# wuliwei9278/primalCR

Measured on AMD Instinct MI355X. Metric: pairwise-comparisons/sec, higher is better.
Workload: dtype f32; 1 GPU; ml1m-shaped PrimalCR++ -k 100 -l 5000 (configs[1]); 6040 users x 3952 items, 939809 ratings, 131347247 ordered pairs; 1 step = 1 outer iteration (V step + U step); solver=PrimalCR++, rank=100, parallelism=user-sharded x1, accumulation=f64, storage=f32

## Files before the change

### primalcr_amd/csrc/pcr_host.cpp

```cpp
#include "pcr_host.h"

#include <algorithm>
#include <atomic>
#include <cerrno>
#include <climits>
#include <cstdint>
#include <cmath>
#include <cstdio>
#include <cstdlib>
#include <cstring>
#include <exception>
#include <functional>
#include <limits>
#include <memory>
#include <mutex>
#include <numeric>
#include <random>
#include <thread>
#include <fcntl.h>
#include <sys/mman.h>
#include <sys/stat.h>
#include <unistd.h>

static thread_local std::string g_err;
// ... 213 lines not shown
}

static int check_test_ids(int64_t d2, int64_t tnnz, const int32_t* tuser, const int32_t* titem, int threads) {
    const int T = pieces_for(tnnz, threads);
    std::vector<int64_t> bad((size_t)T, -1);
    run_pieces(tnnz, T, [&](int t, int64_t lo, int64_t hi) {
        for (int64_t z = lo; z < hi; ++z)
            if (titem[z] < 0 || titem[z] >= d2 || tuser[z] < 0) { bad[(size_t)t] = z; return; }
    });
    for (int64_t b : bad)
        if (b >= 0) {
            pcr_set_error("test rating " + std::to_string(b) + " has user/item id outside the meta dimensions");
            return PCR_ERR_ARG;
        }
    return PCR_OK;
}

extern "C" int pcr_dataset_from_triplets(int64_t d1, int64_t d2, int64_t nnz, const int32_t* user,
                                         const int32_t* item, const double* val, int64_t tnnz,
                                         const int32_t* tuser, const int32_t* titem, const double* tval,
                                         pcr_dataset** out) {
    if (!out || d1 < 0 || d2 < 0 || nnz < 0 || tnnz < 0 || (nnz > 0 && (!user || !item || !val)) ||
        (tnnz > 0 && (!tuser || !titem || !tval))) {
        pcr_set_error("pcr_dataset_from_triplets: bad argument");
        return PCR_ERR_ARG;
    }
    if (d1 > kMaxDim || d2 > kMaxDim) { pcr_set_error("pcr_dataset_from_triplets: more than 2^31 - 2 users or items"); return PCR_ERR_UNSUPPORTED; }
    return guarded("pcr_dataset_from_triplets", [&]() -> int {
        std::unique_ptr<pcr_dataset> ds(new pcr_dataset());
        const int threads = pcr_host_threads();
        int rc = build_train_csr(d1, d2, nnz, user, item, val, ds->train, threads, false);
        if (rc != PCR_OK) return rc;
        rc = check_test_ids(d2, tnnz, tuser, titem, threads);
        if (rc != PCR_OK) return rc;
        keep_raw_test(*ds, d1, tnnz, tuser, titem, tval);
        build_test_csr(d1, d2, tnnz, tuser, titem, tval, ds->test, threads, false);
        ds->tnnz_file = tnnz;
        *out = ds.release();
        return PCR_OK;
    });
}

extern "C" int pcr_dataset_from_csr(int64_t d1, int64_t d2, const int64_t* index, const int32_t* item, const double* val,
                                    const int64_t* tindex, const int32_t* titem, const double* tval, pcr_dataset** out) {
    if (!out || d1 < 0 || d2 < 0 || !index || index[0] != 0 || (tindex && tindex[0] != 0)) {
        pcr_set_error("pcr_dataset_from_csr: bad argument");
        return PCR_ERR_ARG;
    }
    const int64_t nnz = index[d1], tnnz = tindex ? tindex[d1] : 0;
    if (nnz < 0 || tnnz < 0 || (nnz > 0 && (!item || !val)) || (tnnz > 0 && (!titem || !tval))) {
        pcr_set_error("pcr_dataset_from_csr: bad argument");
        return PCR_ERR_ARG;
    }
    for (int64_t u = 0; u < d1; ++u) {
        if (index[u + 1] < index[u] || (tindex && tindex[u + 1] < tindex[u])) { pcr_set_error("pcr_dataset_from_csr: index not monotone"); return PCR_ERR_ARG; }
        for (int64_t z = index[u]; z < index[u + 1]; ++z)
            if (item[z] < 0 || item[z] >= d2 || (z > index[u] && item[z] <= item[z - 1])) {
                pcr_set_error("pcr_dataset_from_csr: user " + std::to_string(u) + ": item ids must be ascending and inside [0, d2)");
                return PCR_ERR_ARG;
            }
    }
    for (int64_t z = 0; z < tnnz; ++z)
        if (titem[z] < 0 || titem[z] >= d2) { pcr_set_error("pcr_dataset_from_csr: test item id outside [0, d2)"); return PCR_ERR_ARG; }
    if (d1 > kMaxDim || d2 > kMaxDim) { pcr_set_error("pcr_dataset_from_csr: more than 2^31 - 2 users or items"); return PCR_ERR_UNSUPPORTED; }
    return guarded("pcr_dataset_from_csr", [&]() -> int {
        std::unique_ptr<pcr_dataset> ds(new pcr_dataset());
        ds->train.d1 = ds->test.d1 = d1; ds->train.d2 = ds->test.d2 = d2;
        ds->train.index.assign(index, index + d1 + 1);
        ds->train.item.assign(item, item + nnz);
        ds->train.val.assign(val, val + nnz);
        if (tindex) ds->test.index.assign(tindex, tindex + d1 + 1); else ds->test.index.assign(d1 + 1, 0);
        ds->test.item.assign(titem, titem + tnnz);
        ds->test.val.assign(tval, tval + tnnz);
        ds->tnnz_file = tnnz;
        *out = ds.release();
        return PCR_OK;
    });
}

#include <map>
static std::map<std::string, std::string>& tune_table() { static thread_local std::map<std::string, std::string> t; return t; }
static const char* const TUNE_KEYS[] = {"ustep_mode", "cluster_k", "cluster_users", "ubins", "ustep_gram", "spmm_tiles", "spmm_chunk", "sddmm_csc",
                                        "lanes", "pipeline", "window_cache", "prepare_merged", "resort_window", "allreduce_chunks", "p2p_ll",
                                        "p2p_timeout_ms", "p2p_queue_budget", "count_rows", "debug", "win16", "ustep_win_lds", "plan_key64", "ustep_newton", "vblock_users", "recommend_select", "ranks_batch_users", "sample_threads", "rerank_lds", "ridge_form", "nnls_form", "itemfold_table_bytes", "fault_cluster_member", "fault_p2p_skip", "fault_p2p_coarse", nullptr};
extern "C" int pcr_tune(const char* key, const char* value) {
    if (!key) { pcr_set_error("pcr_tune: null key"); return PCR_ERR_ARG; }
    bool known = false;
    for (const char* const* k = TUNE_KEYS; *k; ++k) known = known || !strcmp(*k, key);
    if (!known) { pcr_set_error(std::string("pcr_tune: unknown key '") + key + "'"); return PCR_ERR_ARG; }
    if (value) tune_table()[key] = value; else tune_table().erase(key);
    return PCR_OK;
}
bool pcr_tune_get(const char* key, std::string* out) {
    auto it = tune_table().find(key);
    if (it == tune_table().end()) return false;
    if (out) *out = it->second;
    return true;
}
int pcr_tune_int(const char* key, int dflt) {
    std::string v;
    return pcr_tune_get(key, &v) ? atoi(v.c_str()) : dflt;
}


struct TextFile {
    const char* p = nullptr;
    size_t len = 0;
    void* map = nullptr;
    size_t map_len = 0;
    pcr_vec<char> heap;
    ~TextFile() { if (map) munmap(map, map_len); }
    int open(const std::string& path) {
        const int fd = ::open(path.c_str(), O_RDONLY | O_CLOEXEC);
        if (fd < 0) { pcr_set_error("can't open " + path + ": " + strerror(errno)); return PCR_ERR_IO; }
        struct stat sb;
        if (fstat(fd, &sb) == 0 && S_ISREG(sb.st_mode) && sb.st_size > 0) {
            void* m = mmap(nullptr, (size_t)sb.st_size, PROT_READ, MAP_PRIVATE, fd, 0);
            if (m != MAP_FAILED) {
                (void)madvise(m, (size_t)sb.st_size, MADV_WILLNEED);
                map = m; map_len = (size_t)sb.st_size; p = static_cast<const char*>(m); len = map_len;
                ::close(fd);
                return PCR_OK;
            }
        }
        size_t cap = (size_t)1 << 20, got = 0;
        heap.resize(cap);
        for (;;) {
            const ssize_t n = ::read(fd, heap.data() + got, cap - got);
            if (n < 0) { if (errno == EINTR) continue; ::close(fd); pcr_set_error("can't read " + path + ": " + strerror(errno)); return PCR_ERR_IO; }
            if (n == 0) break;
            got += (size_t)n;
            if (got == cap) { cap *= 2; heap.resize(cap); }
        }
        ::close(fd);
        p = heap.data(); len = got;
        return PCR_OK;
    }
};

struct SlowCopy {
    char buf[512];
    size_t n;
    SlowCopy(const char* p, const char* end) { n = std::min<size_t>(sizeof(buf) - 1, (size_t)(end - p)); memcpy(buf, p, n); buf[n] = 0; }
};

static inline bool parse_one(const char*& p, const char* end, int32_t& u, int32_t& it, double& v) {
    auto skip_ws = [&]() { while (p < end && (*p == ' ' || *p == '\t' || *p == '\n' || *p == '\r')) ++p; };
    auto parse_uint = [&](long& out) -> bool {
        skip_ws();
        const char* s = p;
        long x = 0;
        while (p < end && *p >= '0' && *p <= '9') { if (x < ((long)1 << 40)) x = x * 10 + (*p - '0'); ++p; }
        if (p == s || (p < end && (*p == '.' || *p == '-' || *p == '+' || *p == 'e' || *p == 'E'))) { p = s; return false; }
        out = x;
        return true;
    };
    const char* save = p;
    long a, b;
    if (parse_uint(a) && parse_uint(b)) {
        skip_ws();
        const char* s = p;
        bool neg = false;
        if (p < end && (*p == '-' || *p == '+')) { neg = *p == '-'; ++p; }
        long ip = 0; int nd = 0;
        while (p < end && *p >= '0' && *p <= '9' && nd < 15) { ip = ip * 10 + (*p - '0'); ++p; ++nd; }
        bool simple = nd > 0 || (p < end && *p == '.');
        double val = (double)ip;
// ... 1714 lines not shown
```

### primalcr_amd/csrc/pcr_solver.hip

```cpp
#include <hip/hip_runtime.h>
#include <rccl/rccl.h>

#include <algorithm>
#include <chrono>
#include <cmath>
#include <cstdio>
#include <cstring>
#include <limits>
#include <memory>
#include <string>
#include <vector>

#include "pcr_host.h"
#include "pcr_dev.h"
#include "pcr_kernels.h"
#include "pcr_gram.h"
#include "pcr_newton.h"
#include "pcr_vblock.h"
#include "pcr_p2p.h"

#define NCCLCHK(expr)                                                                          \
    do {                                                                                       \
        ncclResult_t e_ = (expr);                                                              \
        if (e_ != ncclSuccess) {                                                               \
            pcr_set_error(std::string(#expr) + ": " + ncclGetErrorString(e_));                 \
            return PCR_ERR_COMM;                                                               \
        }                                                                                      \
    } while (0)
#include "pcr_plan.h"
#include "pcr_plan_dev.h"

#include "pcr_classes.h"

struct Tune {
    int lanes = 0, spmm_chunk = 0, spmm_tiles = 0, sddmm_csc = -1, ustep_mode = 0, cluster_k = 4, cluster_users = 0, window_cache = 1,
        prepare_merged = -1, pipeline = 1, debug = 0, fault_cluster_member = 0, ustep_gram = -1, count_rows = 0, allreduce_chunks = 0,
        resort_window = 8, p2p_ll = 16, p2p_timeout_ms = 20000, p2p_queue_budget = 0, fault_p2p_skip = 0, fault_p2p_coarse = 0, win16 = 1, ustep_win_lds = 1, plan_key64 = 0, ustep_newton = 0, vblock_users = 0, recommend_select = 1;
    std::string ubins;
    void read() {
        lanes = pcr_tune_int("lanes", 0); spmm_chunk = pcr_tune_int("spmm_chunk", 0); spmm_tiles = pcr_tune_int("spmm_tiles", 0);
        sddmm_csc = pcr_tune_int("sddmm_csc", -1); ustep_mode = pcr_tune_int("ustep_mode", 0); cluster_k = pcr_tune_int("cluster_k", 4);
        cluster_users = pcr_tune_int("cluster_users", 0); window_cache = pcr_tune_int("window_cache", 1);
        prepare_merged = pcr_tune_int("prepare_merged", -1);
        pipeline = pcr_tune_int("pipeline", 1); debug = pcr_tune_int("debug", 0); fault_cluster_member = pcr_tune_int("fault_cluster_member", 0);
        ustep_gram = pcr_tune_int("ustep_gram", -1); count_rows = pcr_tune_int("count_rows", 0);
        allreduce_chunks = pcr_tune_int("allreduce_chunks", 0);
        resort_window = pcr_tune_int("resort_window", 8); p2p_ll = pcr_tune_int("p2p_ll", 16);
        p2p_timeout_ms = pcr_tune_int("p2p_timeout_ms", 20000); fault_p2p_skip = pcr_tune_int("fault_p2p_skip", 0);
        fault_p2p_coarse = pcr_tune_int("fault_p2p_coarse", 0); p2p_queue_budget = pcr_tune_int("p2p_queue_budget", 0);
        win16 = pcr_tune_int("win16", 1); ustep_win_lds = pcr_tune_int("ustep_win_lds", 1); plan_key64 = pcr_tune_int("plan_key64", 0); ustep_newton = pcr_tune_int("ustep_newton", 0); vblock_users = pcr_tune_int("vblock_users", 0);
        recommend_select = pcr_tune_int("recommend_select", 1);
        ubins.clear(); pcr_tune_get("ubins", &ubins);
    }
};

template <typename T>
struct Solver final : pcr_solver {
    pcr_params prm;
    Tune tune;
    int rank = 0, nranks = 1;
    int64_t d1 = 0, d2 = 0, tnnz_file = 0;
    Geo geo;
    hipStream_t st = nullptr;
    static constexpr int NSIDE = 12;
    hipStream_t side[NSIDE] = {};
    hipEvent_t ev_fork = nullptr;
    hipStream_t hi = nullptr;
    hipEvent_t ev_hi = nullptr;
    static constexpr int MAXLANE = 8;
    hipStream_t lane[MAXLANE] = {};
    hipEvent_t ev_lane[MAXLANE] = {};
    int nlane = 1;
    int pipe_lanes = 0;
    bool hi_on_solver_pipe = false;
    std::vector<hipStream_t> hi_spare;
    ncclComm_t comm = nullptr;
    std::unique_ptr<P2PComm> p2p;
    bool single() const { return (nranks == 1 && !comm && !p2p) || local_only; }
    int ncu = 256;

    Shard<T> sh;
    DBuf<int64_t> d_uptr, d_runofs;
    DBuf<int32_t> d_sidx;
    DBuf<double> d_objr;
    DBuf<int32_t> d_item, d_c2r, d_runstart, d_sitem, d_cuser, d_crow, d_ruser, d_slot_base, d_item_slot, d_chunk_ptr, d_slot_id;
    DBuf<int2> d_blk_chunks;
    DBuf<int32_t> d_blk_user, d_cpos_dense;
    DBuf<unsigned char> d_excl;
    int vblock_nbp = 0;
    DBuf<int32_t> d_newton_users;
    DBuf<double> d_dir;
    DBuf<char> d_newton_scratch;
    int newton_n = 0, newton_cap = 0, newton_rs = 0, newton_grid = 0;
    size_t newton_stride = 0;
    DBuf<int32_t> d_cuf;
    int spmm_blocks = 0, spmm_tiles = 1;
    int n_rng = 1;
    std::vector<int64_t> rng_item;
    std::vector<int> rng_blk;
    hipStream_t ar_st = nullptr;
    std::vector<hipEvent_t> ev_rng;
    hipEvent_t ev_ar = nullptr;
    bool sddmm_csc = false;
    DBuf<T> d_slab;
    bool sweep_pf4 = false;
    int spmm_chunk = 128;
    int sddmm_tile = 0;
    DBuf<uint16_t> d_lvl, d_slvl;
    DBuf<unsigned char> d_rhint;
    DBuf<uint16_t> d_win;
    DBuf<T> d_ms, d_c, d_mcsr, d_b;
    DBuf<double> d_objp;
    std::vector<Bin> bins;
    std::vector<Bin> sbins;
    std::vector<Bin> pbins;
    std::vector<Bin> ubins;
    unsigned* bar_p = nullptr;
    size_t bar_n = 0;
    DBuf<char> d_xch;
    DBuf<unsigned long long> d_rowcnt;
    size_t xch_stride = 0;
    int max_clusters = 1;
    struct EvalSet {
        int64_t nnz = 0;
        DBuf<int64_t> uptr;
        DBuf<int32_t> item;
        DBuf<double> val, gain, idcg, disc;
        DBuf<uint16_t> elvl;
        DBuf<int64_t> erunofs;
        DBuf<int32_t> erunstart;
        int max_raw_levels = 0;
        std::vector<Bin> bins;
        std::vector<int64_t> h_uptr;
        std::vector<double> h_val;
// ... 702 lines not shown
        for (int l = 1; l < nlane; ++l)
            if (used[l]) { HIPCHK(hipEventRecord(ev_lane[l], lane[l])); RC(join(ev_lane[l])); }
        HIPCHK(hipGetLastError());
        return PCR_OK;
    }
    int join(hipEvent_t ev) {
        if (!device_join) HIPCHK(hipEventSynchronize(ev)); else HIPCHK(hipStreamWaitEvent(st, ev, 0));
        return PCR_OK;
    }
    template <class F>
    int for_ubins(F launch) {
        std::vector<Bin*> order;
        for (auto& b : ubins) if (!b.users.empty() && b.K > 1) order.push_back(&b);
        const size_t nhead = order.size();
        for (auto& b : ubins) if (!b.users.empty() && b.K <= 1) order.push_back(&b);
        if (order.empty()) return PCR_OK;
        std::stable_sort(order.begin() + nhead, order.end(), [](const Bin* a, const Bin* b) { return a->cap > b->cap; });
        std::vector<std::pair<int, int>> plan;
        {
            for (size_t i = 0; i < nhead; ++i) plan.push_back({(int)i, MAXLANE});
            std::vector<int> ring;
            for (int l = 0; l < nlane; ++l) ring.push_back(nlane >= 2 && l < 2 ? l ^ 1 : l);
            std::vector<int> tail_ring;
            for (int l : ring) if (l != 0) { tail_ring.push_back(l); if (tail_ring.size() == 1 && nhead) tail_ring.push_back(MAXLANE); }
            tail_ring.push_back(0);
            for (size_t i = nhead; i < order.size(); ++i) {
                const size_t j = i - nhead;
                plan.push_back({(int)i, j < ring.size() ? ring[j] : tail_ring[(j - ring.size()) % tail_ring.size()]});
            }
        }
        if (tune.debug && !plan_announced && (plan_announced = true))
            for (auto& pr : plan) fprintf(stderr, "[pcr] U step: %s on stream %d\n", pname("ustep", *order[pr.first]).c_str(), pr.second);
        const bool idle = hipStreamQuery(st) == hipSuccess;
        ProfScope wall(&prof, "wall:ustep", st);
        bool used[MAXLANE + 1] = {};
        if (!idle) HIPCHK(hipEventRecord(ev_fork, st));
        for (auto& pr : plan) {
            Bin& b = *order[pr.first];
            hipStream_t q = pr.second == MAXLANE ? hi : lane[pr.second];
            if (!idle && q != st && !used[pr.second]) HIPCHK(hipStreamWaitEvent(q, ev_fork, 0));
            used[pr.second] = true;
            ProfScope ps(&prof, pname("ustep", b), q, b.nnz, (int64_t)b.users.size());
            launch(b, q);
        }
        for (int l = 1; l < nlane; ++l)
            if (used[l]) { HIPCHK(hipEventRecord(ev_lane[l], lane[l])); RC(join(ev_lane[l])); }
        if (used[MAXLANE]) { HIPCHK(hipEventRecord(ev_hi, hi)); RC(join(ev_hi)); }
        HIPCHK(hipGetLastError());
        return PCR_OK;
    }
    bool plan_announced = false;
    template <class F>
    int for_bins_seq(std::vector<Bin>& bs, const char* cls, F launch) {
        for (auto& b : bs) {
            if (b.users.empty()) continue;
            ProfScope ps(&prof, pname(cls, b), st, b.nnz, (int64_t)b.users.size());
            launch(b, st);
        }
        HIPCHK(hipGetLastError());
        return PCR_OK;
    }
    std::string ustep_classes() override {
        std::string all;
        for (auto& b : ubins) if (!b.users.empty()) { if (!all.empty()) all += ","; all += pname("ustep", b); }
        return all;
    }
    int class_rows(const std::string& slot, double* v) override {
        for (size_t bi = 0; bi < ubins.size(); ++bi) {
            if (ubins[bi].users.empty() || pname("ustep", ubins[bi]) != slot) continue;
            unsigned long long x = 0;
            HIPCHK(hipStreamSynchronize(st));
            HIPCHK(hipMemcpy(&x, d_rowcnt.p + bi, sizeof x, hipMemcpyDeviceToHost));
            *v = (double)x;
            return PCR_OK;
        }
        pcr_set_error("pcr_solver_counter: no U-step class '" + slot + "'");
        return PCR_ERR_ARG;
    }
    size_t small_common(int block) const { return carve_bytes(geo.ld, sizeof(T)) + carve_bytes(block / PCR_WAVE + 1, 8); }
    int strict() const { return prm.solver_type == PCR_SOLVER_PCR ? 1 : 0; }
    int foldin_params(pcr_params* p) override { *p = prm; return PCR_OK; }
    double ridge_lambda() override { return prm.lambda; }

    int launch_sddmm(const T* M, const int32_t* rows, T* out, const int* skip = nullptr) {
        if (nnz_local == 0) return PCR_OK;
        ProfScope ps(&prof, "sddmm", st);
        const T* Umat = d_U.p;
        if (sddmm_tile == 0) {
            sddmm_tile = 64;
            int per_cu = 0;
            const int ngrp0 = 256 / geo.G;
            if (hipOccupancyMaxActiveBlocksPerMultiprocessor(&per_cu, k_sddmm<T, 256>, 256, (size_t)ngrp0 * 128 * 8) == hipSuccess && per_cu > 0) {
                const int64_t fit = cdiv(nnz_local, (int64_t)ncu * per_cu * ngrp0);
                if (fit > 64 && fit <= 128) sddmm_tile = (int)((fit + 7) / 8 * 8);
            }
        }
        const int tile = sddmm_tile;
        const int ngrp = 256 / geo.G, span = ngrp * tile;
        const int grid = cdiv(nnz_local, span);
        hipLaunchKernelGGL((k_sddmm<T, 256>), dim3(grid), dim3(256), (size_t)span * 8, st, Umat, M, d_ruser.p, rows, nnz_local, out, geo, tile, skip,
                           (const int32_t*)nullptr, (const int2*)nullptr, (const int32_t*)nullptr);
        HIPCHK(hipGetLastError());
        return PCR_OK;
    }
    bool sddmm_by_tiles() const { return sddmm_csc; }
    int launch_sddmm_csc(const T* A, T* out, const int* skip) {
        if (nnz_local == 0) return PCR_OK;
        ProfScope ps(&prof, "sddmm", st);
        const int span = (256 / geo.G) * spmm_chunk;
        hipLaunchKernelGGL((k_sddmm<T, 256>), dim3(spmm_blocks), dim3(256), (size_t)span * 8, st, A, d_U.p, d_crow.p, d_cuser.p, nnz_local, out, geo,
                           spmm_chunk, skip, d_c2r.p, d_blk_chunks.p, d_chunk_ptr.p);
        HIPCHK(hipGetLastError());
        return PCR_OK;
    }

    bool prepare_is_single_launch() const {
        const bool merged = tune.prepare_merged >= 0 ? tune.prepare_merged != 0 : nnz_local < (int64_t)4000000;
        return merged && !pbins[0].users.empty() && !pbins[1].users.empty();
    }
    int launch_prepare(const T* Vm) {
        RC(launch_sddmm(Vm, d_item.p, d_mcsr.p));
        const Shard<T>& shp = sh;
        auto fn = [&](Bin& b, hipStream_t q) {
            const int nus = (int)b.users.size();
            const int cap_pad = b.big ? host_pow2(b.cap) : b.cap, rsc = b.max_lev + 2;
            const size_t bigb = prepare_bytes<T>(b.cap, cap_pad, rsc, b.big ? 8 : 4);
            const size_t lds = small_common(b.block) + (b.big ? 0 : bigb);
            const int grid = b.big ? std::min(nus, scratch_blocks) : nus;
#define LP(BL, BG) hipLaunchKernelGGL((k_prepare<T, BL, BG>), dim3(grid), dim3(BL), lds, q, shp, geo, b.d_users.p, nus, d_mcsr.p, b.cap, cap_pad, rsc, d_scratch.p, scratch_stride, strict())
            if (b.big) LP(512, true);
            else if (b.block == 64) LP(64, false);
            else if (b.block == 256) LP(256, false);
            else LP(512, false);
#undef LP
        };
        Bin &ba = pbins[0], &bb = pbins[1];
        if (prepare_is_single_launch()) {
            const int na = (int)ba.users.size(), nb = (int)bb.users.size();
            const int cpa = ba.cap, cpb = bb.cap, rsa = ba.max_lev + 2, rsb = bb.max_lev + 2;
            const size_t wb = (small_common(64) + prepare_bytes<T>(ba.cap, cpa, rsa, 4) + 15) & ~(size_t)15;
            const int wbs = 512, wpb = wbs / 64;
            const size_t lds = std::max(wb * wpb, small_common(wbs) + prepare_bytes<T>(bb.cap, cpb, rsb, 4));
            {
                ProfScope ps(&prof, "prepare/all", st, ba.nnz + bb.nnz, (int64_t)(na + nb));
                hipLaunchKernelGGL((k_prepare_all<T, 512>), dim3(nb + cdiv(na, wpb)), dim3(512), lds, st, shp, ba.d_users.p, na, ba.cap, cpa, rsa, wb,
                                   bb.d_users.p, nb, bb.cap, cpb, rsb, nb, d_mcsr.p, strict());
            }
            if (!pbins[2].users.empty()) { ProfScope ps(&prof, pname("prepare", pbins[2]), st, pbins[2].nnz, (int64_t)pbins[2].users.size()); fn(pbins[2], st); }
            HIPCHK(hipGetLastError());
            have_sorted = true;
            sh.prev_valid = 1;
            return PCR_OK;
        }
        RC(for_bins(bins, "prepare", fn));
        have_sorted = true;
        sh.prev_valid = 1;
        return PCR_OK;
    }

    int launch_vsweep(bool hv, const T* A, const int* skip = nullptr) {
        if (hv) { if (sddmm_by_tiles()) RC(launch_sddmm_csc(A, d_b.p, skip)); else RC(launch_sddmm(A, d_sitem.p, d_b.p, skip)); }
        if (hv && vblock_nbp) {
            ProfScope ps(&prof, "vblock_b", st);
            const int64_t tiles = (int64_t)(vblock_nbp / GramMfma<T>::TS) * cdiv(d2, GramMfma<T>::TS);
#ifndef PCR_NO_OPTIONAL_KERNELS
            hipLaunchKernelGGL((k_vblock_b<T>), dim3((unsigned)cdiv(tiles, 4)), dim3(256), 0, st, d_U.p, A, d_blk_user.p, vblock_nbp, d_cpos_dense.p, d2, geo, d_b.p, skip);
#endif
            HIPCHK(hipGetLastError());
        }
        return launch_sweeps(hv, skip, hv && sddmm_by_tiles());
    }
    int launch_sweeps(bool hv, const int* skip, bool b_csr = false) {
        const int bc = (b_csr ? 1 : 0) | (sweep_pf4 ? 2 : 0);
        const bool two = hv && !sh.ws;
        const bool wt = sh.uw != nullptr;
        auto fn = [&](Bin& b, hipStream_t q) {
            const int nus = (int)b.users.size();
            const int rsc = b.max_lev + 2;
            if (b.block == 64) {
                const size_t wb = (vsweep_wave_bytes<T>(b.cap, rsc, two) + 15) & ~(size_t)15;
#define LW(HV, WT) hipLaunchKernelGGL((k_vsweep_wave<T, HV, WT>), dim3(cdiv(nus, 4)), dim3(256), wb * 4, q, sh, b.d_users.p, nus, d_b.p, d_c.p, b.cap, rsc, wb, strict(), skip, bc)
                if (hv) { if (wt) LW(true, true); else LW(true, false); } else { if (wt) LW(false, true); else LW(false, false); }
#undef LW
                return;
            }
            const size_t bigb = vsweep_bytes<T>(b.cap, rsc, two);
            const size_t lds = small_common(b.block) + (b.big ? 0 : bigb);
            const int grid = b.big ? std::min(nus, scratch_blocks) : nus;
#define LV(BL, BG, HV) do { if (wt) LVW(BL, BG, HV, true); else LVW(BL, BG, HV, false); } while (0)
#define LVW(BL, BG, HV, WT) hipLaunchKernelGGL((k_vsweep<T, BL, BG, HV, WT>), dim3(grid), dim3(BL), lds, q, sh, geo, b.d_users.p, nus, d_b.p, d_c.p, b.cap, rsc, d_scratch.p, scratch_stride, strict(), skip, bc)
            if (hv) { if (b.big) LV(512, true, true); else LV(512, false, true); }
            else { if (b.big) LV(512, true, false); else LV(512, false, false); }
#undef LVW
#undef LV
        };
        Bin &ba = sbins[0], &bb = sbins[1];
        if (!ba.users.empty() && !bb.users.empty()) {
            const int na = (int)ba.users.size(), nb = (int)bb.users.size();
            const int rsa = ba.max_lev + 2, rsb = bb.max_lev + 2;
            const size_t wb = (vsweep_wave_bytes<T>(ba.cap, rsa, two) + 15) & ~(size_t)15;
            const int wbs = 512, wpb = wbs / 64;
            const size_t lds = std::max(wb * wpb, small_common(wbs) + vsweep_bytes<T>(bb.cap, rsb, two));
            const int grid = nb + cdiv(na, wpb);
            {
                ProfScope ps(&prof, std::string(hv ? "vhv" : "vgrad") + "/all", st, ba.nnz + bb.nnz, (int64_t)(na + nb));
#define LVA(HV, WBS, MW) do { if (wt) LVAW(HV, WBS, MW, true); else LVAW(HV, WBS, MW, false); } while (0)
#define LVAW(HV, WBS, MW, WT) hipLaunchKernelGGL((k_vsweep_all<T, HV, WBS, MW, WT>), dim3(grid), dim3(WBS), lds, st, sh, ba.d_users.p, na, ba.cap, rsa, wb, \
                                        bb.d_users.p, nb, bb.cap, rsb, nb, d_b.p, d_c.p, strict(), skip, bc)
                const bool dense = lds <= (size_t)40 * 1024;
                if (hv) { if (dense) { LVA(true, 512, 8); } else { LVA(true, 512, 1); } } else { if (dense) { LVA(false, 512, 8); } else { LVA(false, 512, 1); } }
#undef LVAW
#undef LVA
            }
            if (!sbins[2].users.empty()) { ProfScope ps(&prof, pname(hv ? "vhv" : "vgrad", sbins[2]), st, sbins[2].nnz, (int64_t)sbins[2].users.size()); fn(sbins[2], st); }
            HIPCHK(hipGetLastError());
            return PCR_OK;
        }
        RC(for_bins_seq(sbins, hv ? "vhv" : "vgrad", fn));
        return PCR_OK;
    }

    int fin_blocks() const { return (int)std::min<int64_t>(1024, cdiv(d2, 256 / geo.G)); }
    int launch_spmm_range(int r, T* out, const T* base, double beta, const int* skip, const T* dots_rr) {
        if (nnz_local > 0 && rng_blk[r + 1] > rng_blk[r]) {
            ProfScope ps(&prof, "spmm", st);
            hipLaunchKernelGGL((k_spmm<T, 256>), dim3(rng_blk[r + 1] - rng_blk[r]), dim3(256), 0, st, d_c.p, d_c2r.p, d_cuf.p,
                               d_chunk_ptr.p, d_slot_base.p, d_slot_id.p, d_blk_chunks.p + rng_blk[r], d_U.p, d_slab.p, geo, skip);
        }
        const int j0 = (int)rng_item[r], j1 = (int)rng_item[r + 1];
        if (j1 <= j0) return PCR_OK;
        const int grid = n_rng == 1 ? fin_blocks() : (int)std::min<int64_t>(1024, cdiv(j1 - j0, 256 / geo.G));
        ProfScope ps2(&prof, "spmm_fin", st);
        if (dots_rr) hipLaunchKernelGGL((k_spmm_fin<T, 256, true>), dim3(grid), dim3(256), 0, st, d_slab.p, d_item_slot.p, base, beta, j1, out, geo, skip, dots_rr, d_partA.p, j0);
        else hipLaunchKernelGGL((k_spmm_fin<T, 256, false>), dim3(grid), dim3(256), 0, st, d_slab.p, d_item_slot.p, base, beta, j1, out, geo, skip, (const T*)nullptr, (double*)nullptr, j0);
        return PCR_OK;
    }
    int launch_spmm(T* out, const T* base, double beta, const int* skip = nullptr, const T* dots_rr = nullptr) {
        const size_t n = (size_t)d2 * geo.ld;
        if (n_rng == 1) {
            RC(launch_spmm_range(0, out, base, beta, skip, dots_rr));
            if (vblock_nbp) {
                ProfScope ps(&prof, "vblock_hp", st);
                const int64_t tiles = (int64_t)cdiv(d2, GramMfma<T>::TS) * cdiv(geo.ld, GramMfma<T>::TS);
#ifndef PCR_NO_OPTIONAL_KERNELS
                hipLaunchKernelGGL((k_vblock_hp<T>), dim3((unsigned)cdiv(tiles, 4)), dim3(256), 0, st, d_U.p, d_c.p, d_blk_user.p, vblock_nbp, d_cpos_dense.p, d2, geo, out, skip);
#endif
            }
            HIPCHK(hipGetLastError());
            return allreduce_T(out, n);
        }
        const bool exch = !single();
        auto queue = [&](int r) -> int {
            RC(launch_spmm_range(r, out, base, beta, skip, nullptr));
            if (exch) HIPCHK(hipEventRecord(ev_rng[r], st));
            return PCR_OK;
        };
        RC(queue(0));
        for (int r = 0; r < n_rng; ++r) {
            if (r + 1 < n_rng) RC(queue(r + 1));
            if (!exch) continue;
            HIPCHK(hipStreamWaitEvent(ar_st, ev_rng[r], 0));
            const size_t lo = (size_t)rng_item[r] * geo.ld, hi = (size_t)rng_item[r + 1] * geo.ld;
            if (hi > lo) RC(allreduce_T(out + lo, hi - lo, ar_st));
        }
        if (exch) { HIPCHK(hipEventRecord(ev_ar, ar_st)); HIPCHK(hipStreamWaitEvent(st, ev_ar, 0)); }
        HIPCHK(hipGetLastError());
        return PCR_OK;
    }

    int allreduce_T(T* buf, size_t count, hipStream_t q = nullptr) {
        if (single()) return PCR_OK;
        if (!comm && !p2p) { pcr_set_error("nranks > 1 but neither pcr_solver_comm_init nor pcr_solver_comm_init_p2p was called"); return PCR_ERR_STATE; }
        if (!q) q = st;
        ProfScope ps(&prof, "allreduce", q);
        if (p2p) {
            if (!p2p->allreduce<T>(buf, count, q)) { pcr_set_error("p2p all-reduce: " + p2p->err); return PCR_ERR_COMM; }
            return PCR_OK;
        }
        NCCLCHK(ncclAllReduce(buf, buf, count, sizeof(T) == 4 ? ncclFloat : ncclDouble, ncclSum, comm, q));
        return PCR_OK;
    }
    int allreduce_f64(double* buf, size_t count) override {
        if (single()) return PCR_OK;
        if (!comm && !p2p) { pcr_set_error("nranks > 1 but neither pcr_solver_comm_init nor pcr_solver_comm_init_p2p was called"); return PCR_ERR_STATE; }
        ProfScope ps(&prof, "allreduce", st);
        if (p2p) {
            if (!p2p->allreduce<double>(buf, count, st, true)) { pcr_set_error("p2p all-reduce: " + p2p->err); return PCR_ERR_COMM; }
            return PCR_OK;
        }
        NCCLCHK(ncclAllReduce(buf, buf, count, ncclDouble, ncclSum, comm, st));
        return PCR_OK;
    }

    int reduce_sum(const double* in, int64_t n, int slot) {
        const int nb = (int)std::min<int64_t>(512, std::max<int64_t>(1, cdiv(n, 2048)));
        const int per = cdiv(std::max<int64_t>(n, 1), nb);
        hipLaunchKernelGGL(k_sum_stage1, dim3(nb), dim3(PCR_EW_BLOCK), 0, st, in, n, per, d_partA.p);
        hipLaunchKernelGGL(k_fin2, dim3(1), dim3(PCR_EW_BLOCK), 0, st, d_partA.p, nb, d_scal.p + slot);
        HIPCHK(hipGetLastError());
        return PCR_OK;
    }
    int norm2(const T* a, int64_t n, int slot) {
        const int nb = (int)std::min<int64_t>(512, std::max<int64_t>(1, cdiv(n, 4096)));
        const int per = cdiv(std::max<int64_t>(n, 1), nb);
        hipLaunchKernelGGL((k_dots<T>), dim3(nb), dim3(PCR_EW_BLOCK), 0, st, a, (const T*)nullptr, n, per, d_partB.p);
        hipLaunchKernelGGL(k_fin2, dim3(1), dim3(PCR_EW_BLOCK), 0, st, d_partB.p, nb, d_scal.p + slot);
        HIPCHK(hipGetLastError());
        return PCR_OK;
    }
    int sync_checked() {
// ... 861 lines not shown
```

### primalcr_amd/csrc/pcr_vside.h

```cpp
#pragma once
#include "pcr_prims.h"

template <typename T, int BLOCK>
__global__ __launch_bounds__(BLOCK) void k_sddmm(const T* __restrict__ U, const T* __restrict__ M,
                                                 const int32_t* __restrict__ ruser, const int32_t* __restrict__ rows,
                                                 int64_t nnz, T* __restrict__ out, Geo geo, int tile, const int* skip,
                                                 const int32_t* __restrict__ perm, const int2* __restrict__ blk_map,
                                                 const int32_t* __restrict__ chunk_ptr) {
    typedef typename VecOf<T>::type V;
    constexpr int VEC = VecOf<T>::N;
    extern __shared__ __attribute__((aligned(16))) char smem[];
    if (skip && *skip) return;
    const int G = geo.G, g = threadIdx.x & (G - 1), grp = threadIdx.x / G, ngrp = BLOCK / G;
    const int span = ngrp * tile;
    int32_t* s_row = reinterpret_cast<int32_t*>(smem);
    int32_t* s_usr = s_row + span;
    int64_t b0 = (int64_t)blockIdx.x * span;
    int nb = (int)((nnz - b0 < span) ? (nnz - b0) : span);
    if (blk_map) {
        const int2 bc = blk_map[blockIdx.x];
        if (bc.y == 0) return;
        b0 = chunk_ptr[bc.x];
        nb = chunk_ptr[bc.x + bc.y] - (int)b0;
    }
    for (int t = threadIdx.x; t < nb; t += BLOCK) { s_row[t] = rows[b0 + t]; s_usr[t] = ruser[b0 + t]; }
    __syncthreads();
    const int l0 = grp * tile;
    const int l1 = (l0 + tile < nb) ? l0 + tile : nb;
    const int rho = 4 * (g & 1) + (g & 2) + ((g >> 2) & 1);
    for (int k = 0; k * G < geo.nchunk; ++k) {
        const int ch = g + k * G;
        const bool act = ch < geo.nchunk;
        int cur = -1;
        V uv = V{};
        const int chv = act ? ch : 0;
        for (int q0 = l0; q0 < l1; q0 += PCR_UNR) {
            V rv[PCR_UNR];
            T part[PCR_UNR];
            bool fast = false;
            if (q0 + PCR_UNR <= l1) {
                const int4 i0 = *reinterpret_cast<const int4*>(s_row + q0), i1 = *reinterpret_cast<const int4*>(s_row + q0 + 4);
                const int4 u0 = *reinterpret_cast<const int4*>(s_usr + q0), u1 = *reinterpret_cast<const int4*>(s_usr + q0 + 4);
                const int ri[PCR_UNR] = {i0.x, i0.y, i0.z, i0.w, i1.x, i1.y, i1.z, i1.w};
#pragma unroll
                for (int e = 0; e < PCR_UNR; ++e) rv[e] = *reinterpret_cast<const V*>(M + row_off(ri[e], geo) + chv * VEC);
                if (u0.x != cur) {
                    cur = u0.x;
                    uv = *reinterpret_cast<const V*>(U + row_off(cur, geo) + chv * VEC);
                    if (!act) uv = V{};
                }
                fast = (u0.y == cur) & (u0.z == cur) & (u0.w == cur) & (u1.x == cur) & (u1.y == cur) & (u1.z == cur) & (u1.w == cur);
                if (fast) {
#pragma unroll
                    for (int e = 0; e < PCR_UNR; ++e) part[e] = vdot(rv[e], uv);
                } else {
                    const int ui8[PCR_UNR] = {u0.x, u0.y, u0.z, u0.w, u1.x, u1.y, u1.z, u1.w};
#pragma unroll
                    for (int e = 0; e < PCR_UNR; ++e) {
                        if (ui8[e] != cur) {
                            cur = ui8[e];
                            uv = *reinterpret_cast<const V*>(U + row_off(cur, geo) + chv * VEC);
                            if (!act) uv = V{};
                        }
                        part[e] = vdot(rv[e], uv);
                    }
                    fast = true;
                }
            }
            if (!fast) {
#pragma unroll
                for (int e = 0; e < PCR_UNR; ++e)
                    if (q0 + e < l1) rv[e] = *reinterpret_cast<const V*>(M + row_off(s_row[q0 + e], geo) + chv * VEC);
#pragma unroll
                for (int e = 0; e < PCR_UNR; ++e) {
                    part[e] = (T)0;
                    if (q0 + e < l1) {
                        const int uu = s_usr[q0 + e];
                        if (uu != cur) {
                            cur = uu;
                            uv = *reinterpret_cast<const V*>(U + row_off(uu, geo) + chv * VEC);
                            if (!act) uv = V{};
                        }
                        part[e] = vdot(rv[e], uv);
                    }
                }
            }
            if (G >= 8) {
                const T tot = group_reduce8<T>(part, g, G);
                const int q = q0 + rho;
                if (g < 8 && q < l1) { const int64_t o = perm ? (int64_t)perm[b0 + q] : b0 + q; out[o] = (k == 0) ? tot : out[o] + tot; }
            } else {
#pragma unroll
                for (int e = 0; e < PCR_UNR; ++e) {
                    T v = part[e];
                    if (G > 2) v += __shfl_xor(v, 2);
                    if (G > 1) v += __shfl_xor(v, 1);
                    if (g == 0 && q0 + e < l1) { const int64_t o = perm ? (int64_t)perm[b0 + q0 + e] : b0 + q0 + e; out[o] = (k == 0) ? v : out[o] + v; }
                }
            }
        }
    }
}

template <typename T, bool BIG> struct LiSel { typedef uint32_t type; };
template <typename T> struct LiSel<T, true> { typedef uint64_t type; };

template <typename T>
// ... 168 lines not shown
    vsweep_block_body<T, BLOCK, BIG, HV, WT>(smem, S, users, nusers, bsrc, c_out, cap, rs_cap, scratch, stride, strict,
                                         (int)blockIdx.x, (int)gridDim.x, b_csr);
}

template <typename T>
static inline size_t vsweep_wave_bytes(int cap, int rs_cap, bool two) {
    return carve_bytes(cap, sizeof(T)) * (two ? 2 : 1) + carve_bytes(cap + 1, 8) + carve_bytes(rs_cap, 4);
}
template <typename T, bool HV, bool WT = false>
__device__ __forceinline__ void vsweep_wave_body(char* smem, const Shard<T>& S, const int32_t* __restrict__ users, int nusers,
                                                 const T* __restrict__ bsrc, T* __restrict__ c_out,
                                                 int cap, int rs_cap, size_t wave_bytes, int strict, int ui, int flags = 0) {
    const int b_csr = flags & 1, pf4 = flags & 2;
    const int lane = threadIdx.x & 63, wid = threadIdx.x >> 6;
    if (ui >= nusers) return;
    Carver big(smem + (size_t)wid * wave_bytes);
    T* ms = big.take<T>(cap);
    T* x = (HV && !S.ws) ? big.take<T>(cap) : ms;
    double* Sx = big.take<double>(cap + 1);
    int* rs = big.take<int>(rs_cap);
    const int u = users[ui];
    const int64_t s0 = S.uptr[u];
    const int n = (int)(S.uptr[u + 1] - s0);
    const int nlev = (int)(S.runofs[u + 1] - S.runofs[u]) - 1;
    if (n == 0) return;
    double cu = 1.0;
    if constexpr (WT) cu = S.uw[u];
    if (!HV || !S.ws) {
#pragma unroll 4
        for (int p = lane; p < n; p += 64) ms[p] = S.ms[s0 + p];
    }
    for (int l = lane; l <= nlev; l += 64) rs[l] = S.runstart[S.runofs[u] + l];
    const T* xs = ms;
    if (HV) {
#pragma unroll 4
        for (int p = lane; p < n; p += 64) x[p] = bsrc[s0 + (b_csr ? S.sidx[s0 + p] : p)];
        xs = x;
    }
    wave_sync();
    double carry = 0.0;
    for (int base = 0; base < n; base += 64) {
        const int i = base + lane;
        const double v = (i < n) ? (double)xs[i] : 0.0;
        const double inc = wave_incl_scan(v);
        if (i < n) Sx[i] = carry + inc - v;
        carry += lane63(inc);
    }
    if (lane == 0) Sx[n] = carry;
    wave_sync();
    if (S.ws == 4 && S.w16 && pf4) { sweep_out4<T, 64, HV, WT>(S, s0, n, nlev, lane, xs, Sx, rs, c_out, cu); return; }
    for (int p = lane; p < n; p += 64) {
        const int lev = S.slvl[s0 + p];
        const double c = S.ws
            ? sweep_coeff_cached<T>(S, (size_t)(s0 + p), Sx, rs, nlev, lev, (double)xs[p], HV ? 0.0 : 1.0)
            : sweep_coeff<T>(ms, Sx, rs, nlev, lev, ms[p], (double)xs[p], HV ? 0.0 : 1.0, strict);
        c_out[s0 + S.sidx[s0 + p]] = (T)(WT ? c * cu : c);
    }
}
template <typename T, bool HV, bool WT = false>
__global__ __launch_bounds__(256) void k_vsweep_wave(Shard<T> S, const int32_t* __restrict__ users, int nusers,
                                                     const T* __restrict__ bsrc, T* __restrict__ c_out,
                                                     int cap, int rs_cap, size_t wave_bytes, int strict, const int* skip, int b_csr) {
    extern __shared__ __attribute__((aligned(16))) char smem[];
    if (skip && *skip) return;
    vsweep_wave_body<T, HV, WT>(smem, S, users, nusers, bsrc, c_out, cap, rs_cap, wave_bytes, strict,
                            (int)blockIdx.x * 4 + (int)(threadIdx.x >> 6), b_csr);
}

template <typename T, bool HV, int WB, int MINW = 1, bool WT = false>
__global__ __launch_bounds__(WB, MINW) void k_vsweep_all(Shard<T> S, const int32_t* __restrict__ users_a, int nusers_a, int cap_a,
                                                    int rs_cap_a, size_t wave_bytes, const int32_t* __restrict__ users_b,
                                                    int nusers_b, int cap_b, int rs_cap_b, int nblk_b,
                                                    const T* __restrict__ bsrc, T* __restrict__ c_out, int strict, const int* skip, int b_csr) {
    extern __shared__ __attribute__((aligned(16))) char smem[];
    if (skip && *skip) return;
    if ((int)blockIdx.x < nblk_b)
        vsweep_block_body<T, WB, false, HV, WT>(smem, S, users_b, nusers_b, bsrc, c_out, cap_b, rs_cap_b, nullptr, 0, strict,
                                            (int)blockIdx.x, nblk_b, b_csr);
    else
        vsweep_wave_body<T, HV, WT>(smem, S, users_a, nusers_a, bsrc, c_out, cap_a, rs_cap_a, wave_bytes, strict,
                                ((int)blockIdx.x - nblk_b) * (WB / 64) + (int)(threadIdx.x >> 6), b_csr);
}

template <typename T, int BLOCK>
__global__ __launch_bounds__(BLOCK) void k_spmm(const T* __restrict__ c, const int32_t* __restrict__ c2r,
                                                const int32_t* __restrict__ cuf,
                                                const int32_t* __restrict__ chunk_ptr, const int32_t* __restrict__ inc_base,
                                                const int32_t* __restrict__ slot_id, const int2* __restrict__ blk_chunks,
                                                const T* __restrict__ U, T* __restrict__ slab, Geo geo, const int* skip) {
    typedef typename VecOf<T>::type V;
    constexpr int VEC = VecOf<T>::N;
    if (skip && *skip) return;
    const int G = geo.G, g = threadIdx.x & (G - 1);
    const int2 bc = blk_chunks[blockIdx.x];
    if ((int)threadIdx.x / G >= bc.y) return;
    const int gid = bc.x + (int)threadIdx.x / G;
    const int64_t z0 = chunk_ptr[gid], z1 = chunk_ptr[gid + 1];
    for (int k = 0; k * G < geo.nchunk; ++k) {
        const int ch = g + k * G;
        const bool act = ch < geo.nchunk;
        T acc[VEC];
#pragma unroll
        for (int e = 0; e < VEC; ++e) acc[e] = (T)0;
        int inc = inc_base[gid];
        auto flush = [&]() {
            if (act) {
                V o;
                T* op = reinterpret_cast<T*>(&o);
#pragma unroll
                for (int e = 0; e < VEC; ++e) { op[e] = (T)acc[e]; acc[e] = (T)0; }
                {
                    typedef T nat __attribute__((ext_vector_type(VEC)));
                    nat ov;
#pragma unroll
                    for (int e = 0; e < VEC; ++e) ov[e] = op[e];
                    __builtin_nontemporal_store(ov, reinterpret_cast<nat*>(slab + row_off(slot_id[inc], geo) + ch * VEC));
                }
            }
            inc += 1;
        };
        for (int64_t zb = z0; zb < z1; zb += G) {
            const int64_t zi = zb + g;
            T cr = (T)0;
            int ur = 0;
            if (zi < z1) { cr = c2r ? c[c2r[zi]] : c[zi]; ur = cuf[zi]; }
            const int cnt = (int)((z1 - zb < G) ? (z1 - zb) : G);
            for (int q = 0; q < cnt; q += PCR_UNR) {
                V rv[PCR_UNR];
                T cc[PCR_UNR];
                int uf[PCR_UNR];
#pragma unroll
                for (int e8 = 0; e8 < PCR_UNR; ++e8) {
                    if (q + e8 < cnt) {
                        cc[e8] = __shfl(cr, q + e8, G);
                        uf[e8] = __shfl(ur, q + e8, G);
                        if (act) rv[e8] = *reinterpret_cast<const V*>(U + row_off(uf[e8] & 0x7fffffff, geo) + ch * VEC);
                    }
                }
#pragma unroll
                for (int e8 = 0; e8 < PCR_UNR; ++e8) {
                    if (q + e8 < cnt) {
                        if (uf[e8] < 0) flush();
                        if (act) {
#pragma unroll
                            for (int e = 0; e < VEC; ++e) acc[e] += cc[e8] * velem(rv[e8], e);
                        }
                    }
                }
            }
        }
        flush();
    }
}

template <typename T, int BLOCK, bool DOTS>
__global__ __launch_bounds__(BLOCK) void k_spmm_fin(const T* __restrict__ slab, const int32_t* __restrict__ item_slot,
                                                    const T* __restrict__ base, double beta, int d2, T* __restrict__ out,
                                                    Geo geo, const int* skip, const T* __restrict__ rr, double* __restrict__ part,
                                                    int j0 = 0) {
    typedef typename VecOf<T>::type V;
    constexpr int VEC = VecOf<T>::N;
    __shared__ double red[BLOCK / PCR_WAVE + 1];
    if (skip && *skip) return;
    const int G = geo.G, g = threadIdx.x & (G - 1), ipb = BLOCK / G;
    double x = 0.0, y = 0.0, z = 0.0, w = 0.0;
    for (int j = j0 + (int)blockIdx.x * ipb + (int)threadIdx.x / G; j < d2; j += (int)gridDim.x * ipb) {
        const int s0 = item_slot[j], s1 = item_slot[j + 1];
        for (int ch = g; ch < geo.nchunk; ch += G) {
            double acc[VEC];
            const V bv = *reinterpret_cast<const V*>(base + row_off(j, geo) + ch * VEC);
#pragma unroll
            for (int e = 0; e < VEC; ++e) acc[e] = beta * (double)velem(bv, e);
            for (int sl = s0; sl < s1; sl += 8) {
                V pv[8];
#pragma unroll
                for (int q = 0; q < 8; ++q)
                    if (sl + q < s1) pv[q] = *reinterpret_cast<const V*>(slab + row_off(sl + q, geo) + ch * VEC);
#pragma unroll
                for (int q = 0; q < 8; ++q)
                    if (sl + q < s1) {
// ... 204 lines not shown
```

Before: 48.01 billion pairs/s.

## Add 32-bit byte-offset gather SDDMM and prefetching SpMM walk variants

Adds a gather_form tune knob, on by default, that selects new kernel variants when the matrix fits in 32-bit byte offsets and the group width is at least 8. The SDDMM variant precomputes row byte offsets in shared memory so gathers use 32-bit address arithmetic. The SpMM variant double-buffers the coefficient, user and index loads two rounds ahead to hide gather latency, and uses non-temporal stores for slab output. The aim is less address arithmetic and more overlap of dependent loads, at the cost of extra template instantiations and possibly higher register pressure.

```diff
diff --git a/primalcr_amd/csrc/pcr_host.cpp b/primalcr_amd/csrc/pcr_host.cpp
--- a/primalcr_amd/csrc/pcr_host.cpp
+++ b/primalcr_amd/csrc/pcr_host.cpp
@@ -319,7 +319,7 @@
 static std::map<std::string, std::string>& tune_table() { static thread_local std::map<std::string, std::string> t; return t; }
 static const char* const TUNE_KEYS[] = {"ustep_mode", "cluster_k", "cluster_users", "ubins", "ustep_gram", "spmm_tiles", "spmm_chunk", "sddmm_csc",
                                         "lanes", "pipeline", "window_cache", "prepare_merged", "resort_window", "allreduce_chunks", "p2p_ll",
-                                        "p2p_timeout_ms", "p2p_queue_budget", "count_rows", "debug", "win16", "ustep_win_lds", "plan_key64", "ustep_newton", "vblock_users", "recommend_select", "ranks_batch_users", "sample_threads", "rerank_lds", "ridge_form", "nnls_form", "itemfold_table_bytes", "fault_cluster_member", "fault_p2p_skip", "fault_p2p_coarse", nullptr};
+                                        "p2p_timeout_ms", "p2p_queue_budget", "count_rows", "debug", "win16", "ustep_win_lds", "plan_key64", "ustep_newton", "vblock_users", "recommend_select", "gather_form", "ranks_batch_users", "sample_threads", "rerank_lds", "ridge_form", "nnls_form", "itemfold_table_bytes", "fault_cluster_member", "fault_p2p_skip", "fault_p2p_coarse", nullptr};
 extern "C" int pcr_tune(const char* key, const char* value) {
     if (!key) { pcr_set_error("pcr_tune: null key"); return PCR_ERR_ARG; }
     bool known = false;
diff --git a/primalcr_amd/csrc/pcr_solver.hip b/primalcr_amd/csrc/pcr_solver.hip
--- a/primalcr_amd/csrc/pcr_solver.hip
+++ b/primalcr_amd/csrc/pcr_solver.hip
@@ -35,7 +35,7 @@
 struct Tune {
     int lanes = 0, spmm_chunk = 0, spmm_tiles = 0, sddmm_csc = -1, ustep_mode = 0, cluster_k = 4, cluster_users = 0, window_cache = 1,
         prepare_merged = -1, pipeline = 1, debug = 0, fault_cluster_member = 0, ustep_gram = -1, count_rows = 0, allreduce_chunks = 0,
-        resort_window = 8, p2p_ll = 16, p2p_timeout_ms = 20000, p2p_queue_budget = 0, fault_p2p_skip = 0, fault_p2p_coarse = 0, win16 = 1, ustep_win_lds = 1, plan_key64 = 0, ustep_newton = 0, vblock_users = 0, recommend_select = 1;
+        resort_window = 8, p2p_ll = 16, p2p_timeout_ms = 20000, p2p_queue_budget = 0, fault_p2p_skip = 0, fault_p2p_coarse = 0, win16 = 1, ustep_win_lds = 1, plan_key64 = 0, ustep_newton = 0, vblock_users = 0, recommend_select = 1, gather_form = 1;
     std::string ubins;
     void read() {
         lanes = pcr_tune_int("lanes", 0); spmm_chunk = pcr_tune_int("spmm_chunk", 0); spmm_tiles = pcr_tune_int("spmm_tiles", 0);
@@ -49,7 +49,7 @@
         p2p_timeout_ms = pcr_tune_int("p2p_timeout_ms", 20000); fault_p2p_skip = pcr_tune_int("fault_p2p_skip", 0);
         fault_p2p_coarse = pcr_tune_int("fault_p2p_coarse", 0); p2p_queue_budget = pcr_tune_int("p2p_queue_budget", 0);
         win16 = pcr_tune_int("win16", 1); ustep_win_lds = pcr_tune_int("ustep_win_lds", 1); plan_key64 = pcr_tune_int("plan_key64", 0); ustep_newton = pcr_tune_int("ustep_newton", 0); vblock_users = pcr_tune_int("vblock_users", 0);
-        recommend_select = pcr_tune_int("recommend_select", 1);
+        recommend_select = pcr_tune_int("recommend_select", 1); gather_form = pcr_tune_int("gather_form", 1);
         ubins.clear(); pcr_tune_get("ubins", &ubins);
     }
 };
@@ -918,15 +918,22 @@
     int foldin_params(pcr_params* p) override { *p = prm; return PCR_OK; }
     double ridge_lambda() override { return prm.lambda; }
 
+    bool gather_pipe() const {
+        return tune.gather_form != 0 && geo.G >= 8 && (uint64_t)std::max(d1, d2) * (uint64_t)geo.ld * sizeof(T) < ((uint64_t)1 << 32);
+    }
+    bool spmm_ahead() const { return gather_pipe() && sizeof(T) == 4; }
     int launch_sddmm(const T* M, const int32_t* rows, T* out, const int* skip = nullptr) {
         if (nnz_local == 0) return PCR_OK;
         ProfScope ps(&prof, "sddmm", st);
         const T* Umat = d_U.p;
+        const bool pipe = gather_pipe();
         if (sddmm_tile == 0) {
             sddmm_tile = 64;
             int per_cu = 0;
             const int ngrp0 = 256 / geo.G;
-            if (hipOccupancyMaxActiveBlocksPerMultiprocessor(&per_cu, k_sddmm<T, 256>, 256, (size_t)ngrp0 * 128 * 8) == hipSuccess && per_cu > 0) {
+            const hipError_t oq = pipe ? hipOccupancyMaxActiveBlocksPerMultiprocessor(&per_cu, k_sddmm<T, 256, 1>, 256, (size_t)ngrp0 * 128 * 8)
+                                       : hipOccupancyMaxActiveBlocksPerMultiprocessor(&per_cu, k_sddmm<T, 256, 0>, 256, (size_t)ngrp0 * 128 * 8);
+            if (oq == hipSuccess && per_cu > 0) {
                 const int64_t fit = cdiv(nnz_local, (int64_t)ncu * per_cu * ngrp0);
                 if (fit > 64 && fit <= 128) sddmm_tile = (int)((fit + 7) / 8 * 8);
             }
@@ -934,8 +941,10 @@
         const int tile = sddmm_tile;
         const int ngrp = 256 / geo.G, span = ngrp * tile;
         const int grid = cdiv(nnz_local, span);
-        hipLaunchKernelGGL((k_sddmm<T, 256>), dim3(grid), dim3(256), (size_t)span * 8, st, Umat, M, d_ruser.p, rows, nnz_local, out, geo, tile, skip,
-                           (const int32_t*)nullptr, (const int2*)nullptr, (const int32_t*)nullptr);
+        if (pipe) hipLaunchKernelGGL((k_sddmm<T, 256, 1>), dim3(grid), dim3(256), (size_t)span * 8, st, Umat, M, d_ruser.p, rows, nnz_local, out, geo, tile, skip,
+                                     (const int32_t*)nullptr, (const int2*)nullptr, (const int32_t*)nullptr);
+        else hipLaunchKernelGGL((k_sddmm<T, 256, 0>), dim3(grid), dim3(256), (size_t)span * 8, st, Umat, M, d_ruser.p, rows, nnz_local, out, geo, tile, skip,
+                                (const int32_t*)nullptr, (const int2*)nullptr, (const int32_t*)nullptr);
         HIPCHK(hipGetLastError());
         return PCR_OK;
     }
@@ -944,8 +953,10 @@
         if (nnz_local == 0) return PCR_OK;
         ProfScope ps(&prof, "sddmm", st);
         const int span = (256 / geo.G) * spmm_chunk;
-        hipLaunchKernelGGL((k_sddmm<T, 256>), dim3(spmm_blocks), dim3(256), (size_t)span * 8, st, A, d_U.p, d_crow.p, d_cuser.p, nnz_local, out, geo,
-                           spmm_chunk, skip, d_c2r.p, d_blk_chunks.p, d_chunk_ptr.p);
+        if (gather_pipe()) hipLaunchKernelGGL((k_sddmm<T, 256, 1>), dim3(spmm_blocks), dim3(256), (size_t)span * 8, st, A, d_U.p, d_crow.p, d_cuser.p, nnz_local, out, geo,
+                                              spmm_chunk, skip, d_c2r.p, d_blk_chunks.p, d_chunk_ptr.p);
+        else hipLaunchKernelGGL((k_sddmm<T, 256, 0>), dim3(spmm_blocks), dim3(256), (size_t)span * 8, st, A, d_U.p, d_crow.p, d_cuser.p, nnz_local, out, geo,
+                                spmm_chunk, skip, d_c2r.p, d_blk_chunks.p, d_chunk_ptr.p);
         HIPCHK(hipGetLastError());
         return PCR_OK;
     }
@@ -1060,8 +1071,10 @@
     int launch_spmm_range(int r, T* out, const T* base, double beta, const int* skip, const T* dots_rr) {
         if (nnz_local > 0 && rng_blk[r + 1] > rng_blk[r]) {
             ProfScope ps(&prof, "spmm", st);
-            hipLaunchKernelGGL((k_spmm<T, 256>), dim3(rng_blk[r + 1] - rng_blk[r]), dim3(256), 0, st, d_c.p, d_c2r.p, d_cuf.p,
-                               d_chunk_ptr.p, d_slot_base.p, d_slot_id.p, d_blk_chunks.p + rng_blk[r], d_U.p, d_slab.p, geo, skip);
+            if (spmm_ahead()) hipLaunchKernelGGL((k_spmm<T, 256, 1>), dim3(rng_blk[r + 1] - rng_blk[r]), dim3(256), 0, st, d_c.p, d_c2r.p, d_cuf.p,
+                                                  d_chunk_ptr.p, d_slot_base.p, d_slot_id.p, d_blk_chunks.p + rng_blk[r], d_U.p, d_slab.p, geo, skip);
+            else hipLaunchKernelGGL((k_spmm<T, 256, 0>), dim3(rng_blk[r + 1] - rng_blk[r]), dim3(256), 0, st, d_c.p, d_c2r.p, d_cuf.p,
+                                    d_chunk_ptr.p, d_slot_base.p, d_slot_id.p, d_blk_chunks.p + rng_blk[r], d_U.p, d_slab.p, geo, skip);
         }
         const int j0 = (int)rng_item[r], j1 = (int)rng_item[r + 1];
         if (j1 <= j0) return PCR_OK;
diff --git a/primalcr_amd/csrc/pcr_vside.h b/primalcr_amd/csrc/pcr_vside.h
--- a/primalcr_amd/csrc/pcr_vside.h
+++ b/primalcr_amd/csrc/pcr_vside.h
@@ -2,6 +2,85 @@
 #include "pcr_prims.h"
 
 template <typename T, int BLOCK>
+__device__ __forceinline__ void sddmm_walk_off(const T* __restrict__ U, const T* __restrict__ M,
+                                               const int32_t* __restrict__ ruser, const int32_t* __restrict__ rows,
+                                               int64_t b0, int nb, T* __restrict__ out, const Geo& geo, int tile,
+                                               const int32_t* __restrict__ perm, char* smem) {
+    typedef typename VecOf<T>::type V;
+    const int G = geo.G, g = threadIdx.x & (G - 1), grp = threadIdx.x / G, ngrp = BLOCK / G;
+    const int span = ngrp * tile;
+    uint32_t* s_off = reinterpret_cast<uint32_t*>(smem);
+    int32_t* s_usr = reinterpret_cast<int32_t*>(smem) + span;
+    const uint32_t ldb = (uint32_t)geo.ld * (uint32_t)sizeof(T);
+    for (int t = threadIdx.x; t < nb; t += BLOCK) { s_off[t] = (uint32_t)rows[b0 + t] * ldb; s_usr[t] = ruser[b0 + t]; }
+    __syncthreads();
+    const int l0 = grp * tile;
+    const int l1 = (l0 + tile < nb) ? l0 + tile : nb;
+    const int rho = 4 * (g & 1) + (g & 2) + ((g >> 2) & 1);
+    auto dot = [](const V& a, const V& b) -> T {
+        if constexpr (sizeof(T) == 8) return __builtin_fma(a.x, b.x, a.y * b.y); else return vdot(a, b);
+    };
+    auto chunk_at = [](const T* tab, uint32_t byte_off) -> V {
+        return *reinterpret_cast<const V*>(reinterpret_cast<const char*>(tab) + byte_off);
+    };
+    for (int k = 0; k * G < geo.nchunk; ++k) {
+        const int ch = g + k * G;
+        const bool act = ch < geo.nchunk;
+        const uint32_t chb = (uint32_t)(act ? ch : 0) * 16u;
+        int cur = -1;
+        V uv = V{};
+        auto reload = [&](int user) {
+            cur = user;
+            uv = chunk_at(U, (uint32_t)user * ldb + chb);
+            if (!act) uv = V{};
+        };
+        for (int q0 = l0; q0 < l1; q0 += PCR_UNR) {
+            V rv[PCR_UNR];
+            T part[PCR_UNR];
+            bool fast = false;
+            if (q0 + PCR_UNR <= l1) {
+                const uint4 i0 = *reinterpret_cast<const uint4*>(s_off + q0), i1 = *reinterpret_cast<const uint4*>(s_off + q0 + 4);
+                const int4 u0 = *reinterpret_cast<const int4*>(s_usr + q0), u1 = *reinterpret_cast<const int4*>(s_usr + q0 + 4);
+                const uint32_t ro[PCR_UNR] = {i0.x, i0.y, i0.z, i0.w, i1.x, i1.y, i1.z, i1.w};
+#pragma unroll
+                for (int e = 0; e < PCR_UNR; ++e) rv[e] = chunk_at(M, ro[e] + chb);
+                if (u0.x != cur) reload(u0.x);
+                fast = (u0.y == cur) & (u0.z == cur) & (u0.w == cur) & (u1.x == cur) & (u1.y == cur) & (u1.z == cur) & (u1.w == cur);
+                if (fast) {
+#pragma unroll
+                    for (int e = 0; e < PCR_UNR; ++e) part[e] = dot(rv[e], uv);
+                } else {
+                    const int ui8[PCR_UNR] = {u0.x, u0.y, u0.z, u0.w, u1.x, u1.y, u1.z, u1.w};
+#pragma unroll
+                    for (int e = 0; e < PCR_UNR; ++e) {
+                        if (ui8[e] != cur) reload(ui8[e]);
+                        part[e] = dot(rv[e], uv);
+                    }
+                    fast = true;
+                }
+            }
+            if (!fast) {
+#pragma unroll
+                for (int e = 0; e < PCR_UNR; ++e)
+                    if (q0 + e < l1) rv[e] = chunk_at(M, s_off[q0 + e] + chb);
+#pragma unroll
+                for (int e = 0; e < PCR_UNR; ++e) {
+                    part[e] = (T)0;
+                    if (q0 + e < l1) {
+                        const int uu = s_usr[q0 + e];
+                        if (uu != cur) reload(uu);
+                        part[e] = dot(rv[e], uv);
+                    }
+                }
+            }
+            const T tot = group_reduce8<T>(part, g, G);
+            const int q = q0 + rho;
+            if (g < 8 && q < l1) { const int64_t o = perm ? (int64_t)perm[b0 + q] : b0 + q; out[o] = (k == 0) ? tot : out[o] + tot; }
+        }
+    }
+}
+
+template <typename T, int BLOCK, int FORM = 0>
 __global__ __launch_bounds__(BLOCK) void k_sddmm(const T* __restrict__ U, const T* __restrict__ M,
                                                  const int32_t* __restrict__ ruser, const int32_t* __restrict__ rows,
                                                  int64_t nnz, T* __restrict__ out, Geo geo, int tile, const int* skip,
@@ -23,6 +102,7 @@
         b0 = chunk_ptr[bc.x];
         nb = chunk_ptr[bc.x + bc.y] - (int)b0;
     }
+    if constexpr (FORM != 0) { sddmm_walk_off<T, BLOCK>(U, M, ruser, rows, b0, nb, out, geo, tile, perm, smem); return; }
     for (int t = threadIdx.x; t < nb; t += BLOCK) { s_row[t] = rows[b0 + t]; s_usr[t] = ruser[b0 + t]; }
     __syncthreads();
     const int l0 = grp * tile;
@@ -357,7 +437,90 @@
                                 ((int)blockIdx.x - nblk_b) * (WB / 64) + (int)(threadIdx.x >> 6), b_csr);
 }
 
-template <typename T, int BLOCK>
+template <typename T, int BLOCK, bool C2R>
+__device__ __forceinline__ void spmm_walk_ahead(const T* __restrict__ c, const int32_t* __restrict__ c2r,
+                                                const int32_t* __restrict__ cuf, const int32_t* __restrict__ slot_id,
+                                                const T* __restrict__ U, T* __restrict__ slab, const Geo& geo,
+                                                int inc0, int z0, int z1) {
+    typedef typename VecOf<T>::type V;
+    constexpr int VEC = VecOf<T>::N;
+    const int G = geo.G, g = threadIdx.x & (G - 1);
+    const uint32_t ldb = (uint32_t)geo.ld * (uint32_t)sizeof(T);
+    const int nrnd = (z1 - z0 + G - 1) / G;
+    for (int k = 0; k * G < geo.nchunk; ++k) {
+        const int ch = g + k * G;
+        const bool act = ch < geo.nchunk;
+        const uint32_t chb = (uint32_t)(act ? ch : 0) * 16u;
+        T acc[VEC];
+#pragma unroll
+        for (int e = 0; e < VEC; ++e) acc[e] = (T)0;
+        int inc = inc0;
+        int sid = slot_id[inc];
+        auto flush = [&](bool more) {
+            if (act) {
+                typedef T nat __attribute__((ext_vector_type(VEC)));
+                nat ov;
+#pragma unroll
+                for (int e = 0; e < VEC; ++e) { ov[e] = acc[e]; acc[e] = (T)0; }
+                __builtin_nontemporal_store(ov, reinterpret_cast<nat*>(slab + row_off(sid, geo) + ch * VEC));
+            }
+            inc += 1;
+            if (more) sid = slot_id[inc];
+        };
+        auto ld_idx = [&](int r) -> int {
+            const int zi = min(z0 + r * G + g, z1 - 1);
+            return C2R ? c2r[zi] : zi;
+        };
+        auto ld_cu = [&](int r, int idx, T& cv, int& uf) {
+            const int zi = min(z0 + r * G + g, z1 - 1);
+            cv = c[idx]; uf = cuf[zi];
+        };
+        T cra = (T)0, crb = (T)0;
+        int ura = 0, urb = 0, idn = 0;
+        if (z1 > z0) {
+            const int i0 = ld_idx(0), i1 = ld_idx(1);
+            idn = ld_idx(2);
+            ld_cu(0, i0, cra, ura);
+            ld_cu(1, i1, crb, urb);
+        }
+        auto round = [&](T& cr, int& ur, int r) {
+            const int zb = z0 + r * G;
+            const int cnt = (z1 - zb < G) ? (z1 - zb) : G;
+            for (int q = 0; q < cnt; q += PCR_UNR) {
+                V rv[PCR_UNR];
+                T cc[PCR_UNR];
+                int uf[PCR_UNR];
+#pragma unroll
+                for (int e8 = 0; e8 < PCR_UNR; ++e8) {
+                    if (q + e8 < cnt) {
+                        cc[e8] = __shfl(cr, q + e8, G);
+                        uf[e8] = __shfl(ur, q + e8, G);
+                        if (act) rv[e8] = *reinterpret_cast<const V*>(reinterpret_cast<const char*>(U) + ((uint32_t)(uf[e8] & 0x7fffffff) * ldb + chb));
+                    }
+                }
+#pragma unroll
+                for (int e8 = 0; e8 < PCR_UNR; ++e8) {
+                    if (q + e8 < cnt) {
+                        if (uf[e8] < 0) flush(true);
+                        if (act) {
+#pragma unroll
+                            for (int e = 0; e < VEC; ++e) acc[e] += cc[e8] * velem(rv[e8], e);
+                        }
+                    }
+                }
+            }
+            ld_cu(r + 2, idn, cr, ur);
+            idn = ld_idx(r + 3);
+        };
+        for (int r = 0; r < nrnd; r += 2) {
+            round(cra, ura, r);
+            round(crb, urb, r + 1);
+        }
+        flush(false);
+    }
+}
+
+template <typename T, int BLOCK, int FORM = 0>
 __global__ __launch_bounds__(BLOCK) void k_spmm(const T* __restrict__ c, const int32_t* __restrict__ c2r,
                                                 const int32_t* __restrict__ cuf,
                                                 const int32_t* __restrict__ chunk_ptr, const int32_t* __restrict__ inc_base,
@@ -371,6 +534,11 @@
     if ((int)threadIdx.x / G >= bc.y) return;
     const int gid = bc.x + (int)threadIdx.x / G;
     const int64_t z0 = chunk_ptr[gid], z1 = chunk_ptr[gid + 1];
+    if constexpr (FORM != 0) {
+        if (c2r) spmm_walk_ahead<T, BLOCK, true>(c, c2r, cuf, slot_id, U, slab, geo, inc_base[gid], (int)z0, (int)z1);
+        else spmm_walk_ahead<T, BLOCK, false>(c, c2r, cuf, slot_id, U, slab, geo, inc_base[gid], (int)z0, (int)z1);
+        return;
+    }
     for (int k = 0; k * G < geo.nchunk; ++k) {
         const int ch = g + k * G;
         const bool act = ch < geo.nchunk;
```

Measured after the change: 48.05 billion pairs/s, median of 2. About the same (+0.1%).
